# Signalsmith-Audio/signalsmith-stretch

Hardware: AMD Instinct MI355X
Metric: Msamples/sec (in+out) at 48kHz stereo presetDefault (higher is better)
Workload: dtype f32

## Files before the change

### signalsmith-stretch_amd/csrc/smst_fft.hip

```cpp
#include "smst_kernels_common.h"
#include <type_traits>

namespace smst {

template <int SIGN>
__device__ __forceinline__ float2 twiddle(const float2 *__restrict__ tw, int idx) {
	float2 w = tw[idx];
	if (SIGN > 0) w.y = -w.y;
	return w;
}

template <int SIGN>
__device__ __forceinline__ void dft4(float2 &a, float2 &b, float2 &c, float2 &d) {
	float2 apc = cadd(a, c), amc = csub(a, c), bpd = cadd(b, d), bmd = csub(b, d);
	float2 jb = (SIGN < 0) ? mulNegI(bmd) : mulI(bmd);
	a = cadd(apc, bpd);
	b = cadd(amc, jb);
	c = csub(apc, bpd);
	d = csub(amc, jb);
}
template <int SIGN>
__device__ __forceinline__ void dft3(float2 &a, float2 &b, float2 &c) {
	const float s3 = 0.86602540378443864676f;
	float2 bpc = cadd(b, c), bmc = csub(b, c);
	float2 t = make_float2(a.x - 0.5f*bpc.x, a.y - 0.5f*bpc.y);
	float2 u = cscale((SIGN < 0) ? mulNegI(bmc) : mulI(bmc), s3);
	a = cadd(a, bpc);
	b = cadd(t, u);
	c = csub(t, u);
}
template <int SIGN>
__device__ __forceinline__ void dft5(float2 &a, float2 &b, float2 &c, float2 &d, float2 &e) {
	const float c1 = 0.30901699437494742410f, c2 = -0.80901699437494742410f;
	const float s1 = 0.95105651629515357212f, s2 = 0.58778525229247312917f;
	float2 bpe = cadd(b, e), bme = csub(b, e), cpd = cadd(c, d), cmd = csub(c, d);
	float2 t1 = make_float2(a.x + c1*bpe.x + c2*cpd.x, a.y + c1*bpe.y + c2*cpd.y);
	float2 t2 = make_float2(a.x + c2*bpe.x + c1*cpd.x, a.y + c2*bpe.y + c1*cpd.y);
	float2 u1 = make_float2(s1*bme.x + s2*cmd.x, s1*bme.y + s2*cmd.y);
	float2 u2 = make_float2(s2*bme.x - s1*cmd.x, s2*bme.y - s1*cmd.y);
	float2 ju1 = (SIGN < 0) ? mulNegI(u1) : mulI(u1);
	float2 ju2 = (SIGN < 0) ? mulNegI(u2) : mulI(u2);
	a = cadd(a, cadd(bpe, cpd));
	b = cadd(t1, ju1);
	c = cadd(t2, ju2);
	d = csub(t2, ju2);
	e = csub(t1, ju1);
}
template <int SIGN>
__device__ float2 *fftLds(float2 *src, float2 *dst, const FftPlan &plan, const float2 *__restrict__ tw) {
	const int H = plan.H;
	int nCur = H;
	int shift = 0;
	for (int pass = 0; pass < plan.npass; ++pass) {
		const int r = plan.radix[pass];
		const int m = nCur/r;
		const int nb = H/r;
		const int twScale = H/nCur;
		if (r == 4) {
			const int s = 1 << shift;
			for (int t = threadIdx.x; t < nb; t += blockDim.x) {
				const int p = t >> shift, q0 = t & (s - 1);
				const float2 *in = src + q0 + (p << shift);
				const int inStride = m << shift;
				float2 *out = dst + q0 + ((4*p) << shift);
				float2 a = in[0], b = in[inStride], c = in[2*inStride], e = in[3*inStride];
				dft4<SIGN>(a, b, c, e);
				const int ti = p*twScale;
				out[0] = a;
				out[s] = cmulPlain(b, twiddle<SIGN>(tw, ti));
				out[2*s] = cmulPlain(c, twiddle<SIGN>(tw, 2*ti));
				out[3*s] = cmulPlain(e, twiddle<SIGN>(tw, 3*ti));
			}
			shift += 2;
		} else if (r == 2) {
			const int s = 1 << shift;
			for (int t = threadIdx.x; t < nb; t += blockDim.x) {
				const int p = t >> shift, q0 = t & (s - 1);
				const float2 *in = src + q0 + (p << shift);
				const int inStride = m << shift;
				float2 *out = dst + q0 + ((2*p) << shift);
				float2 a = in[0], b = in[inStride];
				out[0] = cadd(a, b);
				out[s] = cmulPlain(csub(a, b), twiddle<SIGN>(tw, p*twScale));
			}
			shift += 1;
		} else if (r == 3) {
			const int s = nb;
			for (int t = threadIdx.x; t < nb; t += blockDim.x) {
				float2 a = src[t], b = src[t + s], c = src[t + 2*s];
				dft3<SIGN>(a, b, c);
				dst[t] = a;
				dst[t + s] = b;
				dst[t + 2*s] = c;
			}
		} else {
			const int s = nb;
			for (int t = threadIdx.x; t < nb; t += blockDim.x) {
				float2 a = src[t], b = src[t + s], c = src[t + 2*s], e = src[t + 3*s], f = src[t + 4*s];
				dft5<SIGN>(a, b, c, e, f);
				dst[t] = a;
				dst[t + s] = b;
				dst[t + 2*s] = c;
				dst[t + 3*s] = e;
				dst[t + 4*s] = f;
			}
		}
		__syncthreads();
		float2 *tmp = src; src = dst; dst = tmp;
		nCur = m;
	}
	return src;
}

template <int SIGN>
__device__ __forceinline__ float2 mulConst(float2 v, float re, float im) {
	const float s = (SIGN < 0) ? -im : im;
	return make_float2(v.x*re - v.y*s, v.x*s + v.y*re);
}
template <int SIGN>
__device__ __forceinline__ void dft16(float2 (&v)[16]) {
#pragma unroll
	for (int i = 0; i < 4; ++i) dft4<SIGN>(v[i], v[i + 4], v[i + 8], v[i + 12]);
	const float c1 = 0.92387953251128675613f, s1 = 0.38268343236508977173f, h = 0.70710678118654752440f;
	v[1 + 4] = mulConst<SIGN>(v[1 + 4], c1, s1);
	v[1 + 8] = mulConst<SIGN>(v[1 + 8], h, h);
	v[1 + 12] = mulConst<SIGN>(v[1 + 12], s1, c1);
	v[2 + 4] = mulConst<SIGN>(v[2 + 4], h, h);
	v[2 + 8] = (SIGN < 0) ? mulNegI(v[2 + 8]) : mulI(v[2 + 8]);
	v[2 + 12] = mulConst<SIGN>(v[2 + 12], -h, h);
	v[3 + 4] = mulConst<SIGN>(v[3 + 4], s1, c1);
	v[3 + 8] = mulConst<SIGN>(v[3 + 8], -h, h);
	v[3 + 12] = mulConst<SIGN>(v[3 + 12], -c1, -s1);
#pragma unroll
	for (int e = 0; e < 4; ++e) dft4<SIGN>(v[4*e], v[4*e + 1], v[4*e + 2], v[4*e + 3]);
}
template <int SIGN, int RA, int N>
__device__ __forceinline__ void dftPow2(float2 (&v)[N], int base, int stride) {
	if constexpr (RA == 2) {
		const float2 a = v[base], b = v[base + stride];
		v[base] = cadd(a, b);
		v[base + stride] = csub(a, b);
	} else if constexpr (RA == 4) {
		dft4<SIGN>(v[base], v[base + stride], v[base + 2*stride], v[base + 3*stride]);
	} else {
		static_assert(RA == 8, "radix 2, 4 or 8");
		float2 e0 = v[base], e1 = v[base + 2*stride], e2 = v[base + 4*stride], e3 = v[base + 6*stride];
		float2 o0 = v[base + stride], o1 = v[base + 3*stride], o2 = v[base + 5*stride], o3 = v[base + 7*stride];
		dft4<SIGN>(e0, e1, e2, e3);
		dft4<SIGN>(o0, o1, o2, o3);
		const float h = 0.70710678118654752440f;
		o1 = mulConst<SIGN>(o1, h, h);
		o2 = (SIGN < 0) ? mulNegI(o2) : mulI(o2);
		o3 = mulConst<SIGN>(o3, -h, h);
		v[base] = cadd(e0, o0); v[base + 4*stride] = csub(e0, o0);
		v[base + stride] = cadd(e1, o1); v[base + 5*stride] = csub(e1, o1);
		v[base + 2*stride] = cadd(e2, o2); v[base + 6*stride] = csub(e2, o2);
		v[base + 3*stride] = cadd(e3, o3); v[base + 7*stride] = csub(e3, o3);
	}
}
template <int R3> struct LastStage {
	static constexpr int G = (R3%3 == 0) ? 3 : 5;
	static constexpr int RA = R3/G;
	static_assert(R3%G == 0 && (RA == 2 || RA == 4 || RA == 8), "last stage: {2,4,8} x {3,5} points");
};
template <int SIGN, int R3>
__device__ __forceinline__ void dftLast(float2 (&v)[R3]) {
	constexpr int G = LastStage<R3>::G, RA = LastStage<R3>::RA;
#pragma unroll
	for (int i = 0; i < G; ++i) dftPow2<SIGN, RA>(v, i, G);
#pragma unroll
	for (int i = 1; i < G; ++i) {
#pragma unroll
		for (int e = 1; e < RA; ++e) {
			const float ang = 6.28318530717958647692f*float(i*e)/float(R3);
			v[i + G*e] = mulConst<SIGN>(v[i + G*e], __builtin_cosf(ang), __builtin_sinf(ang));
		}
	}
#pragma unroll
	for (int e = 0; e < RA; ++e) {
		if constexpr (G == 3) dft3<SIGN>(v[G*e], v[G*e + 1], v[G*e + 2]);
		else dft5<SIGN>(v[G*e], v[G*e + 1], v[G*e + 2], v[G*e + 3 < R3 ? G*e + 3 : 0], v[G*e + 4 < R3 ? G*e + 4 : 0]);
	}
}

struct BlockSync { __device__ __forceinline__ void operator()() const { __syncthreads(); } };
struct NoHook { __device__ __forceinline__ void operator()() const {} };
struct NoArrival { __device__ __forceinline__ float2 operator()(float2 v, int) const { return v; } };
template <int SIGN, int R3, bool LEAN, int ROUNDS = 0, typename Load, typename Prep, typename Store, typename Sync = BlockSync, typename LastRead = NoHook,
          typename Requested = NoHook, typename FirstWritten = NoHook, typename Arrived = NoArrival>
__device__ __forceinline__ void fftFast(float2 *lds, const float4 *__restrict__ twA, const float4 *__restrict__ twB, Load load, Prep prep, Store store,
                                        const int t = threadIdx.x, Sync sync = Sync(), LastRead lastRead = LastRead(), Requested requested = Requested(),
                                        FirstWritten firstWritten = FirstWritten(), Arrived arrived = Arrived()) {
	constexpr int MA = 16*R3;
	float2 v[16];
	if (t < MA) {
#pragma unroll
		for (int k = 0; k < 16; ++k) v[k] = load(t + MA*k, k);
	}
	requested();
	if (t < MA) {
#pragma unroll
		for (int k = 0; k < 16; ++k) v[k] = arrived(v[k], t + MA*k);
		float2 w[16];
		if constexpr (LEAN) {
			const float4 a = twA[t], b = twA[MA + t], c = twA[2*MA + t];
			const float sg = (SIGN > 0) ? -1.0f : 1.0f;
			w[1] = make_float2(a.x, sg*a.y); w[2] = make_float2(a.z, sg*a.w); w[3] = make_float2(b.x, sg*b.y); w[4] = make_float2(b.z, sg*b.w);
			w[8] = make_float2(c.x, sg*c.y); w[12] = make_float2(c.z, sg*c.w);
#pragma unroll
			for (int hi = 4; hi <= 12; hi += 4) {
#pragma unroll
				for (int lo = 1; lo < 4; ++lo) w[hi + lo] = cmulPlain(w[hi], w[lo]);
			}
		} else {
			float4 wA[8];
#pragma unroll
			for (int i = 0; i < 8; ++i) wA[i] = twA[i*MA + t];
#pragma unroll
			for (int n = 1; n < 16; ++n) {
				const float4 pr = wA[(n - 1) >> 1];
				w[n] = ((n - 1) & 1) ? make_float2(pr.z, pr.w) : make_float2(pr.x, pr.y);
				if (SIGN > 0) w[n].y = -w[n].y;
			}
		}
		dft16<SIGN>(v);
#pragma unroll
		for (int pos = 0; pos < 16; ++pos) {
			const int n = (pos >> 2) + 4*(pos & 3);
			float2 val = v[pos];
			if (n > 0) val = cmulPlain(val, w[n]);
			lds[17*t + n] = val;
		}
	}
	firstWritten();
	sync();
	const int p = t >> 4, q0 = t & 15;
	if (t < MA) {
#pragma unroll
		for (int k = 0; k < 16; ++k) v[k] = lds[q0 + 17*(p + R3*k)];
	}
	sync();
	if (t < MA) {
		float4 wB[8];
#pragma unroll
		for (int i = 0; i < 8; ++i) wB[i] = twB[i*R3 + p];
		dft16<SIGN>(v);
#pragma unroll
		for (int pos = 0; pos < 16; ++pos) {
			const int n = (pos >> 2) + 4*(pos & 3);
			float2 val = v[pos];
			if (n > 0) {
				const float4 pr = wB[(n - 1) >> 1];
				float2 w = ((n - 1) & 1) ? make_float2(pr.z, pr.w) : make_float2(pr.x, pr.y);
				if (SIGN > 0) w.y = -w.y;
				val = cmulPlain(val, w);
			}
			lds[q0 + 256*p + 16*n] = val;
		}
	}
	sync();
	if (t < 256) {
		constexpr int G = LastStage<R3>::G, RA = LastStage<R3>::RA;
		float2 u[R3];
#pragma unroll
		for (int k = 0; k < R3; ++k) u[k] = lds[t + 256*k];
		lastRead();
		constexpr int CHUNK = ROUNDS ? R3/ROUNDS : (R3 <= 12 ? R3 : (R3 == 24 ? 6 : 5));
		decltype(prep(0, 0)) ready[CHUNK];
#pragma unroll
		for (int i = 0; i < CHUNK; ++i) {
			const int e = i/G, c = i - G*e;
			ready[i] = prep(t + 256*(e + RA*c), e + RA*c);
		}
		dftLast<SIGN, R3>(u);
#pragma unroll
		for (int p0 = 0; p0 < R3; p0 += CHUNK) {
			if (p0 > 0) {
#pragma unroll
				for (int i = 0; i < CHUNK; ++i) {
					const int pos = p0 + i, e = pos/G, c = pos - G*e;
					if (pos < R3) ready[i] = prep(t + 256*(e + RA*c), e + RA*c);
				}
			}
#pragma unroll
			for (int i = 0; i < CHUNK; ++i) {
				const int pos = p0 + i, e = pos/G, c = pos - G*e;
				if (pos < R3) store(t + 256*(e + RA*c), u[pos], ready[i], e + RA*c);
			}
		}
	}
}

constexpr int fastBlockThreads(int R3) { return 16*R3 > 256 ? 16*R3 : 256; }

__device__ __forceinline__ bool hopWantsAnalysis(const HopDesc &hd, int which) {
	return (hd.flags & HOP_ACTIVE) && (hd.flags & HOP_NEW_SPECTRUM) && !(hd.flags & HOP_PREANALYSED) && (!which || (hd.flags & HOP_REANALYSE_PREV));
}

__device__ __forceinline__ int halfBinIndex(int j, int H, int N) {
	const int kk = 2*j;
	return kk >= H ? N - 1 - kk : kk;
}
__device__ __forceinline__ float2 loadHalfBin(const float2 *X, int j, int H, int N) {
	float2 v = X[halfBinIndex(j, H, N)];
	if (2*j >= H) v.y = -v.y;
	return v;
}
__device__ __forceinline__ void storeHalfBin(float2 *dst, int j, float2 u, int H, int N) {
	const int kk = 2*j;
	if (kk < H) dst[kk] = u;
	else dst[N - 1 - kk] = cconj(u);
}

__device__ __forceinline__ float2 analysisElement(float4 w, const float *x0, const float *x1, int m, int slot) {
	float2 r = make_float2(0.f, 0.f);
	if (slot < 15) { const float xr = x0[m]; r = make_float2(xr*w.x, xr*w.y); }
	if (slot > 0) { const float xi = x1[m]; r = make_float2(fmaf(xi, w.z, r.x), fmaf(xi, w.w, r.y)); }
	return r;
}
__device__ __forceinline__ float2 leanModulation(float2 hb, int k, int per) {
	const float ang = 3.14159265358979323846f*float(k)/float(per);
	return cmulPlain(hb, make_float2(__builtin_cosf(ang), -__builtin_sinf(ang)));
}
__device__ __forceinline__ void storeWindowed(float *dst, int m, float2 u, float2 tw, float wRe, float wIm, int B, int H) {
	const int halfB = B/2;
	const float2 v = cmulcPlain(u, tw);
	if (m < B - halfB) dst[m + halfB] = (2*v.x)*wRe;
	if (m >= H - halfB) dst[m - H + halfB] = (2*v.y)*wIm;
}
__device__ __forceinline__ void storeWindowed(float *dst, int m, float2 u, float4 r, int B, int H) {
	storeWindowed(dst, m, u, make_float2(r.x, r.y), r.z, r.w, B, H);
}

template <int R3, bool LEAN>
__global__ __launch_bounds__(fastBlockThreads(R3)) __attribute__((amdgpu_waves_per_eu(4, 4))) void kAnalyseFast(DevBatch d, IoArgs io, int sBase, int hopBase, int lateOnly) {
	extern __shared__ __attribute__((aligned(16))) unsigned char smemRaw[];
	float2 *lds = reinterpret_cast<float2 *>(smemRaw);
	const BlockCoord bc = xcdAwareBlock();
	const int k = bc.x;
	const int c = bc.y >> 1;
	const int which = bc.y & 1;
	const int s = bc.s;
	const HopDesc hd = d.hops[(size_t)(sBase + s)*d.hopStride + hopBase + k];
	if (!hopWantsAnalysis(hd, which)) return;
	if (lateOnly && analysisWindowInCall(d.B, d.M, d.I, hd.inputOffset, which, io.inSamples[sBase + s])) return;
	const int B = d.B, H = d.M, halfB = B/2, N = d.N;
	const int base = hd.inputOffset - (which ? d.I : 0) - B;
	const float *x = io.in + (size_t)(sBase + s)*io.inStreamStride + (size_t)c*io.inChannelStride;
	const float *hist = d.hist + ((size_t)(sBase + s)*d.C + c)*(size_t)d.histPitch + d.histBase[d.histCur][sBase + s] + d.histLen;
	const float2 *__restrict__ winA = d.winA, *__restrict__ winB = d.winB;
	float2 *dst = (which ? d.Xprev : d.Xcur) + rowOf(d, s, k, c);
	auto prep = [](int, int) { return 0; };
	auto store = [&](int j, float2 u, int, int) { storeHalfBin(dst, j, u, H, N); };
	constexpr int MA = 16*R3;
	const float4 *__restrict__ twA = LEAN ? d.twA6 : d.twA4;
	const float2 *__restrict__ win2 = d.win2;
	const float2 hb = LEAN ? d.halfTw[min((int)threadIdx.x, MA - 1)] : make_float2(0.f, 0.f);
	if (base >= 0 && H - halfB == MA && B - halfB == 15*MA) {
		const float *x0 = x + base + halfB, *x1 = x + base - H + halfB;
		const float4 *__restrict__ win4 = d.win4;
		fftFast<-1, R3, LEAN>(lds, twA, d.twB4,
			[&](int m, int slot) {
				if constexpr (LEAN) {
					const float2 w = win2[m];
					float2 z = make_float2(0.f, 0.f);
					if (slot < 15) z.x = x0[m]*w.x;
					if (slot > 0) z.y = x1[m]*w.y;
					return cmulPlain(z, leanModulation(hb, slot, 32));
				} else {
					return analysisElement(win4[m], x0, x1, m, slot);
				}
			}, prep, store);
		return;
	}
	fftFast<-1, R3, LEAN>(lds, twA, d.twB4,
		[&](int m, int slot) {
			float xr = 0, xi = 0;
			if (m < B - halfB) { int src = base + m + halfB; xr = (src >= 0) ? x[src] : hist[src]; }
			if (m >= H - halfB) { int src = base + m - H + halfB; xi = (src >= 0) ? x[src] : hist[src]; }
			if constexpr (LEAN) {
				const float2 w = win2[m];
				return cmulPlain(make_float2(xr*w.x, xi*w.y), leanModulation(hb, slot, 32));
			} else {
				const float2 a = winA[m], b = winB[m];
				return make_float2(fmaf(xi, b.x, xr*a.x), fmaf(xi, b.y, xr*a.y));
			}
		}, prep, store);
}

struct TeamSync {
	volatile int *word;
	int *generation;
	__device__ __forceinline__ void operator()() const {
		asm volatile("" ::: "memory");
		__builtin_amdgcn_wave_barrier();
		if ((threadIdx.x & 63) == 0) (void)__hip_atomic_fetch_add(const_cast<int *>(word), 1, __ATOMIC_RELAXED, __HIP_MEMORY_SCOPE_WORKGROUP);
		*generation += 4;
		while (__hip_atomic_load(const_cast<int *>(word), __ATOMIC_RELAXED, __HIP_MEMORY_SCOPE_WORKGROUP) < *generation) __builtin_amdgcn_s_sleep(1);
		__builtin_amdgcn_wave_barrier();
		asm volatile("" ::: "memory");
	}
};
template <int R3, int TEAMS>
struct TeamWorkgroup {
	static_assert(16*R3 <= 256, "a team is 256 threads");
	static constexpr int MA = 16*R3, H = 256*R3;
	float4 *table, *twA, *twB;
	float2 *lds;
	int team, t;
	volatile int *word;
	int generation = 0;
	__device__ __forceinline__ TeamWorkgroup(unsigned char *smem, const DevBatch &d, const float4 *__restrict__ source) {
		team = __builtin_amdgcn_readfirstlane(threadIdx.x >> 8);
		t = threadIdx.x & 255;
		table = reinterpret_cast<float4 *>(smem);
		twA = table + H;
		twB = twA + 8*MA;
		lds = reinterpret_cast<float2 *>(twB + 8*R3) + (size_t)team*(H + H/16);
		volatile int *words = reinterpret_cast<volatile int *>(reinterpret_cast<float2 *>(twB + 8*R3) + (size_t)TEAMS*(H + H/16));
		for (int i = threadIdx.x; i < H; i += blockDim.x) table[i] = source[i];
		for (int i = threadIdx.x; i < 8*MA; i += blockDim.x) twA[i] = d.twA4[i];
		for (int i = threadIdx.x; i < 8*R3; i += blockDim.x) twB[i] = d.twB4[i];
		if (threadIdx.x < 16) words[threadIdx.x] = 0;
		__syncthreads();
		word = words + team;
	}
	TeamWorkgroup(const TeamWorkgroup &) = delete;
	__device__ __forceinline__ TeamSync sync() { return TeamSync{word, &generation}; }
};

template <int R3, int TEAMS, bool EXACT>
__global__ __launch_bounds__(256*TEAMS) void kAnalyseTeams(DevBatch d, IoArgs io, const HopDesc *__restrict__ hopTable, int sBase, int hopBase, int tileHops, int nStreams) {
	extern __shared__ __attribute__((aligned(16))) unsigned char smemRaw[];
	constexpr int MA = 16*R3, H = 256*R3, N = 2*H;
	const int B = EXACT ? 480*R3 : d.B, halfB = B/2;
	const int total = tileHops*2*d.C*nStreams;
	TeamWorkgroup<R3, TEAMS> wg(smemRaw, d, d.win4);
	const TeamSync sync = wg.sync();
	const int t = wg.t, tA = t < MA ? t : 0;
	const int stride = gridDim.x*TEAMS;
	for (int lin = blockIdx.x + gridDim.x*wg.team; lin < total; lin += stride) {
		const BlockCoord bc = xcdAwareCoord(lin, tileHops, 2*d.C, nStreams);
		const HopDesc hd = hopTable[(size_t)(sBase + bc.s)*d.hopStride + hopBase + bc.x];
		const int c = bc.y >> 1, which = bc.y & 1;
		if (!hopWantsAnalysis(hd, which) || !analysisWindowInCall(B, H, d.I, hd.inputOffset, which, io.inSamples[sBase + bc.s])) continue;
		const int base = hd.inputOffset - (which ? d.I : 0) - B;
		const float *x = io.in + (size_t)(sBase + bc.s)*io.inStreamStride + (size_t)c*io.inChannelStride;
		const float *x0 = x + base + halfB, *x1 = x + base - H + halfB;
		float2 *dst = (which ? d.Xprev : d.Xcur) + rowOf(d, bc.s, bc.x, c);
		fftFast<-1, R3, false>(wg.lds, wg.twA, wg.twB,
			[&](int m, int slot) { return analysisElement(wg.table[tA + MA*slot], x0, x1, m, slot); },
			[](int, int) { return 0; },
			[&](int j, float2 u, int, int) { storeHalfBin(dst, j, u, H, N); }, t, sync);
		sync();
	}
}

template <int R3, bool LEAN>
__global__ __launch_bounds__(fastBlockThreads(R3)) void kSynthFast(DevBatch d, int sBase, int hopBase) {
	extern __shared__ __attribute__((aligned(16))) unsigned char smemRaw[];
	float2 *lds = reinterpret_cast<float2 *>(smemRaw);
	const int k = blockIdx.x, c = blockIdx.y, s = blockIdx.z;
	const HopDesc hd = d.hops[(size_t)(sBase + s)*d.hopStride + hopBase + k];
	if (!(hd.flags & HOP_ACTIVE)) return;
	const int B = d.B, H = d.M, N = d.N;
	const float2 *X = d.OUT + rowOf(d, s, k, c);
	float *__restrict__ frame = frameOf(d, s, k, c);
	auto loadBin = [&](int j, int) { return loadHalfBin(X, j, H, N); };
	if constexpr (LEAN) {
		const float2 *__restrict__ win2 = d.win2;
		const float2 hb = d.halfTw[min((int)threadIdx.x, 255)];
		fftFast<+1, R3, true>(lds, d.twA6, d.twB4, loadBin,
			[&](int m, int) { return win2[m]; },
			[&](int m, float2 u, float2 w, int j) { storeWindowed(frame, m, u, leanModulation(hb, j, 2*R3), w.x, w.y, B, H); });
	} else {
		const float4 *__restrict__ synTab = d.synTab;
		fftFast<+1, R3, false>(lds, d.twA4, d.twB4, loadBin,
			[&](int m, int) {
				return synTab[m];
			},
			[&](int m, float2 u, float4 r, int) { storeWindowed(frame, m, u, r, B, H); });
	}
}

template <int R3, int TEAMS>
__global__ __launch_bounds__(256*TEAMS) void kSynthTeams(DevBatch d, const HopDesc *__restrict__ hopTable, int sBase, int hopBase, int tileHops, int nStreams) {
	extern __shared__ __attribute__((aligned(16))) unsigned char smemRaw[];
	constexpr int H = 256*R3, N = 2*H;
	const int B = d.B;
	const int total = tileHops*d.C*nStreams;
	TeamWorkgroup<R3, TEAMS> wg(smemRaw, d, d.synTab);
	const TeamSync sync = wg.sync();
	const int stride = gridDim.x*TEAMS;
	for (int lin = blockIdx.x + gridDim.x*wg.team; lin < total; lin += stride) {
		const BlockCoord bc = xcdAwareCoord(lin, tileHops, d.C, nStreams);
		const HopDesc hd = hopTable[(size_t)(sBase + bc.s)*d.hopStride + hopBase + bc.x];
		if (!(hd.flags & HOP_ACTIVE)) continue;
		const float2 *X = d.OUT + rowOf(d, bc.s, bc.x, bc.y);
		float *__restrict__ frame = frameOf(d, bc.s, bc.x, bc.y);
		fftFast<+1, R3, false>(wg.lds, wg.twA, wg.twB,
			[&](int j, int) { return loadHalfBin(X, j, H, N); },
			[&](int m, int) { return wg.table[m]; },
			[&](int m, float2 u, float4 r, int) { storeWindowed(frame, m, u, r, B, H); }, wg.t, sync);
		sync();
	}
}

__device__ __forceinline__ float carriedSumAt(const DevBatch &d, size_t row, int i) { return i < d.carryLen ? loadCarrySum(d, d.carryCur, row + i) : 0.0f; }
__device__ __forceinline__ float carriedProductAt(const DevBatch &d, const float *__restrict__ carryWpOld, int i) { return i < d.carryLen ? carryWpOld[i] : 1e-30f; }
struct FrameRange { int lo, hi; };
__device__ __forceinline__ FrameRange coveringFrames(int relFirst, int relLast, int B, int I, int hopCount) {
	FrameRange r;
	r.hi = (relLast >= 0) ? relLast/I : -1;
	r.lo = (relFirst - B + 1 > 0) ? (relFirst - B + 1 + I - 1)/I : 0;
	if (r.hi > hopCount - 1) r.hi = hopCount - 1;
	return r;
}
__device__ __forceinline__ float windowProductAt(const DevBatch &d, const EmitDesc &ed, const float *__restrict__ carryWpOld, int i) {
	float wp = carriedProductAt(d, carryWpOld, i);
	if (ed.hopCount > 0) {
		const int rel = ed.nLo + i - ed.firstHopPos - d.delta;
		const FrameRange q = coveringFrames(rel, rel, d.B, d.I, ed.hopCount);
		for (int k = q.lo; k <= q.hi; ++k) wp += d.wprod[rel - k*d.I];
	}
	return wp;
}
__global__ __launch_bounds__(256) void kEmitProducts(DevBatch d, int sBase, int tileIndex) {
	const int sg = sBase + blockIdx.y;
	const EmitDesc ed = d.emit[(size_t)sg*d.emitStride + tileIndex];
	const int span = ed.nHi - ed.nLo, CL = d.carryLen;
	const float *carryWpOld = d.carryWp[d.carryCur] + carryWpRow(d, sg) + d.carryBase[d.carryCur][sg];
	const int i = blockIdx.x*blockDim.x + threadIdx.x;
	if (i == 0) d.carryBase[d.carryCur ^ 1][sg] = 0;
	if (i < d.wpHeadLen) d.wpHead[(size_t)sg*d.wpHeadLen + i] = windowProductAt(d, ed, carryWpOld, i);
	else if (i - d.wpHeadLen < CL) d.carryWp[d.carryCur ^ 1][carryWpRow(d, sg) + (i - d.wpHeadLen)] = windowProductAt(d, ed, carryWpOld, span + (i - d.wpHeadLen));
}

template <int R3, int QN, int SLOTS, bool SPLIT>
__global__ __launch_bounds__(512) void kSynthEmitTeams(DevBatch d, IoArgs io, int sBase, int tileIndex, int nStreams) {
	constexpr int TEAMS = 2, MA = 16*R3, H = 256*R3, N = 2*H, NI = QN + 1, DQ = SPLIT ? 1 : 0;
	extern __shared__ __attribute__((aligned(16))) unsigned char smemRaw[];
	const int B = d.B, I = d.I, CL = d.carryLen;
	TeamWorkgroup<R3, TEAMS> wg(smemRaw, d, d.synTab);
	const TeamSync sync = wg.sync();
	const int team = wg.team, t = wg.t;
	float2 *lds = wg.lds;
	float *ex = reinterpret_cast<float *>(lds);
	float steady[SLOTS];
#pragma unroll
	for (int slot = 0; slot < SLOTS; ++slot) {
		const int r = 256*slot + t;
		steady[slot] = 1e-30f;
#pragma unroll
		for (int a = QN - 1; a >= 0; --a) {
			if (r < I && a*I + r < B) steady[slot] += d.wprod[a*I + r];
		}
		keepUnconditional(steady[slot]);
	}
	const int items = nStreams*d.C;
	for (int item = blockIdx.x*TEAMS + team; item < items; item += gridDim.x*TEAMS) {
		const int s = item/d.C, c = item - s*d.C, sg = sBase + s;
		const EmitDesc ed = d.emit[(size_t)sg*d.emitStride + tileIndex];
		const int cnt = ed.hopCount, span = ed.nHi - ed.nLo;
		const int carryFrom = d.carryBase[d.carryCur][sg];
		const size_t carryRow = carrySumRow(d, sg, c), carried = carryRow + carryFrom;
		const float *wpOld = d.carryWp[d.carryCur] + carryWpRow(d, sg) + carryFrom;
		const float *wpHead = d.wpHead + (size_t)sg*d.wpHeadLen;
		float *out = io.out + (size_t)sg*io.outStreamStride + (size_t)c*io.outChannelStride;
		auto place = [&](int n, float sum, float wp) {
			if (n < ed.nHi) out[n] = sum/wp;
			else if (n - ed.nHi < CL) storeCarrySum(d, d.carryCur ^ 1, carryRow + (n - ed.nHi), sum);
		};
		if (cnt == 0) {
			for (int i = t; i < span + CL; i += 256) place(ed.nLo + i, carriedSumAt(d, carried, i), carriedProductAt(d, wpOld, i));
			continue;
		}
		const int off = ed.firstHopPos - ed.nLo;
		for (int i = t; i < off; i += 256) place(ed.nLo + i, carriedSumAt(d, carried, i), carriedProductAt(d, wpOld, i));
		float acc[NI][SLOTS];
#pragma unroll
		for (int u = 0; u < NI; ++u) {
#pragma unroll
			for (int slot = 0; slot < SLOTS; ++slot) {
				const int r = 256*slot + t, i = off + u*I + r;
				acc[u][slot] = r < I ? carriedSumAt(d, carried, i) : 0.0f;
			}
		}
#pragma unroll
		for (int u = 0; u < NI; ++u) {
#pragma unroll
			for (int slot = 0; slot < SLOTS; ++slot) keepUnconditional(acc[u][slot]);
		}
		auto overlapAdd = [&]() {
			float e[QN][SLOTS];
			int tt = t;
			keepUnconditional(tt);
#pragma unroll
			for (int a = 0; a < QN; ++a) {
#pragma unroll
				for (int slot = 0; slot < SLOTS; ++slot) {
					const int r = 256*slot + tt, i = a*I + r;
					e[a][slot] = ex[r < I && i < B ? i : 0];
				}
			}
#pragma unroll
			for (int a = 0; a < QN; ++a) {
#pragma unroll
				for (int slot = 0; slot < SLOTS; ++slot) {
					const int r = 256*slot + t, i = a*I + r;
					keepUnconditional(e[a][slot]);
					acc[a + DQ][slot] = (r < I && i < B) ? acc[a + DQ][slot] + e[a][slot] : acc[a + DQ][slot];
				}
			}
		};
		auto emitInterval = [&](int q) {
			const int n0 = ed.firstHopPos + q*I;
			float wp[SLOTS];
#pragma unroll
			for (int slot = 0; slot < SLOTS; ++slot) wp[slot] = steady[slot];
			if (q < NI) {
				Async4 head[SLOTS];
#pragma unroll
				for (int slot = 0; slot < SLOTS; ++slot) {
					const int r = 256*slot + t;
					asyncLoad4(head[slot], wpHead + (r < I ? off + q*I + r : 0));
				}
				asyncWait<0>();
#pragma unroll
				for (int slot = 0; slot < SLOTS; ++slot) {
					asyncArrived(head[slot]);
					if (256*slot + t < I) wp[slot] = asyncValue(head[slot]);
				}
			}
			if (n0 + I <= ed.nHi) {
#pragma unroll
				for (int slot = 0; slot < SLOTS; ++slot) {
					const int r = 256*slot + t;
					if (r < I) out[n0 + r] = acc[0][slot]/wp[slot];
				}
			} else {
#pragma unroll
				for (int slot = 0; slot < SLOTS; ++slot) {
					const int r = 256*slot + t;
					if (r < I) place(n0 + r, acc[0][slot], wp[slot]);
				}
			}
#pragma unroll
			for (int u = 0; u + 1 < NI; ++u) {
#pragma unroll
				for (int slot = 0; slot < SLOTS; ++slot) acc[u][slot] = acc[u + 1][slot];
			}
#pragma unroll
			for (int slot = 0; slot < SLOTS; ++slot) acc[NI - 1][slot] = 0.0f;
		};
		Async8 next[16];
#pragma unroll
		for (int k = 0; k < 16; ++k) asyncClear(next[k]);
		auto request = [&](int q) {
			const float2 *X = d.OUT + rowOf(d, s, q, c);
			if (t < MA) {
#pragma unroll
				for (int k = 0; k < 16; ++k) asyncLoad8(next[k], X + halfBinIndex(t + MA*k, H, N));
			}
		};
		auto landed = [&]() {
			asyncWait<0>();
#pragma unroll
			for (int k = 0; k < 16; ++k) asyncArrived(next[k]);
		};
		request(0);
		landed();
		for (int q = 0; q < cnt; ++q) {
			fftFast<+1, R3, false, 2>(lds, wg.twA, wg.twB,
				[&](int, int k) { return asyncValue(next[k]); },
				[&](int m, int) { return wg.table[m]; },
				[&](int m, float2 u, float4 r, int) { storeWindowed(ex, m, u, r, B, H); }, t, sync, sync,
				[&]() {
					if (q > 0) overlapAdd();
					sync();
				},
				[&]() {
					if (q > 0) emitInterval(q - 1);
					request(q + 1 < cnt ? q + 1 : q);
				},
				[&](float2 v, int j) { if (2*j >= H) v.y = -v.y; return v; });
			sync();
			landed();
		}
		overlapAdd();
		sync();
		emitInterval(cnt - 1);
		const bool trailing = SPLIT && ed.firstHopPos + cnt*I < ed.nHi;
		if (trailing) emitInterval(cnt);
		const int n0 = ed.firstHopPos + (cnt + (trailing ? 1 : 0))*I;
#pragma unroll
		for (int u = 0; u < NI; ++u) {
#pragma unroll
			for (int slot = 0; slot < SLOTS; ++slot) {
				const int r = 256*slot + t;
				if (r < I) place(n0 + u*I + r, acc[u][slot], 1.0f);
			}
		}
	}
}

__global__ __launch_bounds__(256) void kEnergy(DevBatch d, IoArgs io, int sBase, float *__restrict__ energyOut) {
	const int s = blockIdx.x, part = blockIdx.y, parts = gridDim.y;
	if (part == 0 && (int)threadIdx.x >= parts && (int)threadIdx.x < kEnergyParts) energyOut[(size_t)(sBase + s)*kEnergyParts + threadIdx.x] = 0.0f;
	const int n = io.inSamples[sBase + s];
	const int lo = (int)((long long)n*part/parts), hi = (int)((long long)n*(part + 1)/parts);
	float acc = 0;
	for (int c = 0; c < d.C; ++c) {
		const float *x = io.in + (size_t)(sBase + s)*io.inStreamStride + (size_t)c*io.inChannelStride;
		for (int i = lo + threadIdx.x; i < hi; i += blockDim.x) {
			float v = x[i];
			acc += v*v;
		}
	}
	extern __shared__ __attribute__((aligned(16))) unsigned char smemRaw[];
	float *red = reinterpret_cast<float *>(smemRaw);
	red[threadIdx.x] = acc;
	__syncthreads();
	for (int w = 128; w > 0; w >>= 1) {
		if ((int)threadIdx.x < w) red[threadIdx.x] += red[threadIdx.x + w];
		__syncthreads();
	}
	if (threadIdx.x == 0) energyOut[(size_t)(sBase + s)*kEnergyParts + part] = red[0];
}

template <bool BIG>
__global__ __launch_bounds__(256) void kAnalyse(DevBatch d, IoArgs io, int sBase, int hopBase) {
	extern __shared__ __attribute__((aligned(16))) unsigned char smemRaw[];
	float2 *bufA = reinterpret_cast<float2 *>(smemRaw);
	float2 *bufB = bufA + d.M;

	const BlockCoord bc = xcdAwareBlock();
	const int k = bc.x;
	const int c = bc.y >> 1;
	const int which = bc.y & 1;
	const int s = bc.s;
	const HopDesc hd = d.hops[(size_t)(sBase + s)*d.hopStride + hopBase + k];
	if (!hopWantsAnalysis(hd, which)) return;

	const int B = d.B, H = d.M, halfB = B/2;
	const int base = hd.inputOffset - (which ? d.I : 0) - B;
	const float *x = io.in + (size_t)(sBase + s)*io.inStreamStride + (size_t)c*io.inChannelStride;
	const float *hist = d.hist + ((size_t)(sBase + s)*d.C + c)*(size_t)d.histPitch + d.histBase[d.histCur][sBase + s];
	const float *__restrict__ win = d.window;
	float2 *dst = (which ? d.Xprev : d.Xcur) + rowOf(d, s, k, c);
	if (BIG) bufB = dst;

	for (int m = threadIdx.x; m < H; m += blockDim.x) {
		float re = 0, im = 0;
		if (m < B - halfB) {
			int i = m + halfB;
			int src = base + i;
			float v = (src >= 0) ? x[src] : hist[d.histLen + src];
			re = v*win[i];
		}
		if (m >= H - halfB) {
			int i = m - H + halfB;
			int src = base + i;
			float v = (src >= 0) ? x[src] : hist[d.histLen + src];
			im = v*win[i];
		}
		bufA[m] = cmulPlain(make_float2(re, im), d.halfTw[m]);
	}
	__syncthreads();
	float2 *res = fftLds<-1>(bufA, bufB, d.plan, d.twH);
	if (BIG && res == dst) {
		for (int j = threadIdx.x; j < H; j += blockDim.x) bufA[j] = dst[j];
		__syncthreads();
		res = bufA;
	}
	const int N = d.N;
	for (int j = threadIdx.x; j < H; j += blockDim.x) storeHalfBin(dst, j, res[j], H, N);
}

template <bool BIG>
__global__ __launch_bounds__(256) void kSynth(DevBatch d, int sBase, int hopBase) {
	extern __shared__ __attribute__((aligned(16))) unsigned char smemRaw[];
	float2 *bufA = reinterpret_cast<float2 *>(smemRaw);
	float2 *bufB = bufA + d.M;
	const int k = blockIdx.x, c = blockIdx.y, s = blockIdx.z;
	if (BIG) bufB = d.fftScratch + rowOf(d, s, k, c);
	const HopDesc hd = d.hops[(size_t)(sBase + s)*d.hopStride + hopBase + k];
	if (!(hd.flags & HOP_ACTIVE)) return;
	const int B = d.B, H = d.M, N = d.N, halfB = B/2;
	const float2 *X = d.OUT + rowOf(d, s, k, c);
	for (int j = threadIdx.x; j < H; j += blockDim.x) bufA[j] = loadHalfBin(X, j, H, N);
	__syncthreads();
	float2 *res = fftLds<+1>(bufA, bufB, d.plan, d.twH);
	float *frame = frameOf(d, s, k, c);
	const float *__restrict__ win = d.window;
	for (int m = threadIdx.x; m < H; m += blockDim.x) {
		const float wRe = (m < B - halfB) ? win[m + halfB] : 0.0f, wIm = (m >= H - halfB) ? win[m - H + halfB] : 0.0f;
		storeWindowed(frame, m, res[m], d.halfTw[m], wRe, wIm, B, H);
	}
}

template <int KMAX>
__global__ __launch_bounds__(256) void kEmit(DevBatch d, IoArgs io, int sBase, int tileIndex) {
	const int s = blockIdx.z, sg = sBase + s, c = blockIdx.y;
	const EmitDesc ed = d.emit[(size_t)sg*d.emitStride + tileIndex];
	const int span = ed.nHi - ed.nLo;
	const int i0 = 4*(blockIdx.x*blockDim.x + threadIdx.x);
	const int CL = d.carryLen;
	const int total = span + CL;
	if (i0 >= total) return;
	const int B = d.B, I = d.I;
	const int carryFrom = d.carryBase[d.carryCur][sg];
	const size_t carryRow = carrySumRow(d, sg, c);
	const float *carryWpOld = d.carryWp[d.carryCur] + carryWpRow(d, sg) + carryFrom;
	if (i0 == 0 && c == 0) d.carryBase[d.carryCur ^ 1][sg] = 0;
	float sum[4], wp[4];
	if (i0 + 3 < CL && !d.halfState) {
		const float4 a = *reinterpret_cast<const float4 *>(d.carrySum[d.carryCur] + carryRow + carryFrom + i0), b = *reinterpret_cast<const float4 *>(carryWpOld + i0);
		sum[0] = a.x; sum[1] = a.y; sum[2] = a.z; sum[3] = a.w;
		wp[0] = b.x; wp[1] = b.y; wp[2] = b.z; wp[3] = b.w;
	} else {
#pragma unroll
		for (int j = 0; j < 4; ++j) {
			const int i = i0 + j;
			sum[j] = carriedSumAt(d, carryRow + carryFrom, i);
			wp[j] = carriedProductAt(d, carryWpOld, i);
		}
	}
	if (ed.hopCount > 0) {
		const int rel0 = ed.nLo + i0 - ed.firstHopPos - d.delta;
		const FrameRange cover = coveringFrames(rel0, rel0 + 3, B, I, ed.hopCount);
		const int qLo = cover.lo, qHi = cover.hi;
		float4 f[KMAX], w[KMAX];
		bool fast[KMAX];
#pragma unroll
		for (int k = 0; k < KMAX; ++k) {
			const int q = qLo + k, idx0 = rel0 - q*I;
			fast[k] = q <= qHi && idx0 >= 0 && idx0 + 3 < B;
			const float *frame = frameOf(d, s, fast[k] ? q : 0, c);
			f[k] = *reinterpret_cast<const float4 *>(frame + (fast[k] ? idx0 : 0));
			w[k] = *reinterpret_cast<const float4 *>(d.wprod + (fast[k] ? idx0 : 0));
		}
#pragma unroll
		for (int k = 0; k < KMAX; ++k) {
			const int q = qLo + k, idx0 = rel0 - q*I;
			if (fast[k]) {
				sum[0] += f[k].x; sum[1] += f[k].y; sum[2] += f[k].z; sum[3] += f[k].w;
				wp[0] += w[k].x; wp[1] += w[k].y; wp[2] += w[k].z; wp[3] += w[k].w;
			} else if (q <= qHi) {
				const float *frame = frameOf(d, s, q, c);
#pragma unroll
				for (int j = 0; j < 4; ++j) {
					const int idx = idx0 + j;
					if (idx >= 0 && idx < B) { sum[j] += frame[idx]; wp[j] += d.wprod[idx]; }
				}
			}
		}
		for (int q = qLo + KMAX; q <= qHi; ++q) {
			const int idx0 = rel0 - q*I;
			const float *frame = frameOf(d, s, q, c);
#pragma unroll
			for (int j = 0; j < 4; ++j) {
				const int idx = idx0 + j;
				if (idx >= 0 && idx < B) { sum[j] += frame[idx]; wp[j] += d.wprod[idx]; }
			}
		}
	}
	float *out = io.out + (size_t)sg*io.outStreamStride + (size_t)c*io.outChannelStride + ed.nLo;
	if (i0 + 3 < span) {
		*reinterpret_cast<float4 *>(out + i0) = make_float4(sum[0]/wp[0], sum[1]/wp[1], sum[2]/wp[2], sum[3]/wp[3]);
	} else {
#pragma unroll
		for (int j = 0; j < 4; ++j) {
			const int i = i0 + j;
			if (i < span) {
				out[i] = sum[j]/wp[j];
			} else if (i < total) {
				storeCarrySum(d, d.carryCur ^ 1, carryRow + (i - span), sum[j]);
				if (c == 0) d.carryWp[d.carryCur ^ 1][carryWpRow(d, sg) + (i - span)] = wp[j];
			}
		}
	}
}

__global__ __launch_bounds__(256) void kEmitCarried(DevBatch d, IoArgs io) {
	const int sg = blockIdx.x;
	const EmitDesc ed = d.emit[(size_t)sg*d.emitStride];
	const int span = ed.nHi - ed.nLo, from = d.carryBase[d.carryCur][sg];
	const float *wpRow = d.carryWp[d.carryCur] + carryWpRow(d, sg) + from;
	for (int c = 0; c < d.C; ++c) {
		const size_t row = carrySumRow(d, sg, c) + from;
		float *out = io.out + (size_t)sg*io.outStreamStride + (size_t)c*io.outChannelStride + ed.nLo;
		for (int i = threadIdx.x; i < span; i += blockDim.x) {
			out[i] = carriedSumAt(d, row, i)/carriedProductAt(d, wpRow, i);
		}
	}
	__syncthreads();
	if (threadIdx.x == 0) d.carryBase[d.carryCur][sg] = from + span;
}

void launchEnergy(const DevBatch &d, const IoArgs &io, int sBase, int nStreams, int maxSamples, float *energyOut, hipStream_t st) {
	const int parts = std::max(1, std::min(kEnergyParts, maxSamples/1024));
	hipLaunchKernelGGL(kEnergy, dim3(nStreams, parts), dim3(256), 256*sizeof(float), st, d, io, sBase, energyOut);
}
template <int... R3S, typename F>
static bool withR3(int M, F f) { return ((M == 256*R3S && (f(std::integral_constant<int, R3S>()), true)) || ...); }
template <typename F> static bool withFastR3(int M, F f) { return withR3<10, 12, 20, 24>(M, f); }
template <typename F> static bool withTeamR3(int M, F f) { return withR3<10, 12>(M, f); }
template <typename F>
static void withFlag(bool flag, F f) {
	if (flag) f(std::true_type()); else f(std::false_type());
}
static size_t fastLdsBytes(int M) { return ((size_t)M + M/16)*sizeof(float2); }
static size_t teamLdsBytes(int M, int teams) {
	return ((size_t)M + M/2 + M/32)*sizeof(float4) + teams*fastLdsBytes(M) + 64;
}
static bool fastApplies(const DevBatch &d) { return !d.noFastFft && isFastSize(d.M); }
static bool teamsAvailable(const DevBatch &d) { return fastApplies(d) && withTeamR3(d.M, [](auto) {}) && d.fftTeams && !d.fftLean; }
static bool teamsApply(const DevBatch &d, int jobs) { return teamsAvailable(d) && (d.fftTeams == 2 || jobs >= 6*d.teamsGrid); }
static int teamsWorkgroups(const DevBatch &d, int jobs) {
	return std::max(8, std::min((jobs + 2)/3/8*8, d.teamsGrid));
}
constexpr int synthEmitQN(int R3) { return R3 == 10 ? 3 : 4; }
constexpr int synthEmitSlots(int R3) { return R3 == 10 ? 8 : 6; }

void launchAnalyse(const DevBatch &d, const IoArgs &io, int sBase, int nStreams, int hopBase, int tileHops, bool anyInCall, bool anyLate, hipStream_t st) {
	const dim3 grid(tileHops, d.C*2, nStreams);
	const int jobs = tileHops*d.C*2*nStreams;
	const bool teams = anyInCall && teamsApply(d, jobs);
	if (teams) {
		const WindowPad pad = windowPad(d.B, d.M);
		withTeamR3(d.M, [&](auto r3) { withFlag(pad.lo == 0 && pad.hi == 0, [&](auto exact) {
			hipLaunchKernelGGL((kAnalyseTeams<r3.value, 3, exact.value>), dim3(teamsWorkgroups(d, jobs)), dim3(768), teamLdsBytes(d.M, 3), st, d, io, d.hops, sBase, hopBase, tileHops, nStreams);
		}); });
		countLaunch(LK_ANALYSE_TEAMS);
		if (!anyLate) return;
	}
	const int lateOnly = teams ? 1 : 0;
	countLaunch(fastApplies(d) ? LK_ANALYSE_FAST : LK_ANALYSE_GENERIC);
	if (!d.noFastFft && withFastR3(d.M, [&](auto r3) { withFlag(d.fftLean != 0, [&](auto lean) {
			hipLaunchKernelGGL((kAnalyseFast<r3.value, lean.value>), grid, dim3(fastBlockThreads(r3.value)), fastLdsBytes(d.M), st, d, io, sBase, hopBase, lateOnly);
		}); })) return;
	size_t lds = 2*(size_t)d.M*sizeof(float2);
	if (fftNeedsScratch(d.M)) hipLaunchKernelGGL(kAnalyse<true>, grid, dim3(256), lds/2, st, d, io, sBase, hopBase);
	else hipLaunchKernelGGL(kAnalyse<false>, grid, dim3(256), lds, st, d, io, sBase, hopBase);
}
void launchSynth(const DevBatch &d, int sBase, int nStreams, int hopBase, int tileHops, hipStream_t st) {
	const dim3 grid(tileHops, d.C, nStreams);
	const int jobs = tileHops*d.C*nStreams;
	if (teamsApply(d, jobs)) {
		withTeamR3(d.M, [&](auto r3) {
			hipLaunchKernelGGL((kSynthTeams<r3.value, 3>), dim3(teamsWorkgroups(d, jobs)), dim3(768), teamLdsBytes(d.M, 3), st, d, d.hops, sBase, hopBase, tileHops, nStreams);
		});
		countLaunch(LK_SYNTH_TEAMS);
		return;
	}
	countLaunch(fastApplies(d) ? LK_SYNTH_FAST : LK_SYNTH_GENERIC);
	if (!d.noFastFft && withFastR3(d.M, [&](auto r3) { withFlag(d.fftLean != 0, [&](auto lean) {
			hipLaunchKernelGGL((kSynthFast<r3.value, lean.value>), grid, dim3(fastBlockThreads(r3.value)), fastLdsBytes(d.M), st, d, sBase, hopBase);
		}); })) return;
	size_t lds = 2*(size_t)d.M*sizeof(float2);
	if (fftNeedsScratch(d.M)) hipLaunchKernelGGL(kSynth<true>, grid, dim3(256), lds/2, st, d, sBase, hopBase);
	else hipLaunchKernelGGL(kSynth<false>, grid, dim3(256), lds, st, d, sBase, hopBase);
}
bool synthEmitApplies(const DevBatch &d, int nStreams, int tileHops) {
	if (!teamsAvailable(d) || !d.synthEmit) return false;
	if (!(d.delta == 0 || d.delta == d.I)) return false;
	const int QN = synthEmitQN(d.M/256), SLOTS = synthEmitSlots(d.M/256);
	if (QN*d.I < d.B || d.I > 256*SLOTS || d.B > d.N) return false;
	if ((QN + 2)*d.I > d.wpHeadLen) return false;
	return d.synthEmit == 2 || (tileHops >= 8 && nStreams*d.C >= 64);
}
void launchEmitProducts(const DevBatch &d, int sBase, int nStreams, int tileIndex, hipStream_t st) {
	hipLaunchKernelGGL(kEmitProducts, dim3(divUp(d.wpHeadLen + d.carryLen, 256), nStreams), dim3(256), 0, st, d, sBase, tileIndex);
}
void launchSynthEmit(const DevBatch &d, const IoArgs &io, int sBase, int nStreams, int tileIndex, hipStream_t st) {
	const int items = nStreams*d.C;
	const int wgs = std::min(divUp(items, 2), d.teamsGrid);
	withTeamR3(d.M, [&](auto r3) { withFlag(d.delta != 0, [&](auto split) {
		hipLaunchKernelGGL((kSynthEmitTeams<r3.value, synthEmitQN(r3.value), synthEmitSlots(r3.value), split.value>), dim3(wgs), dim3(512), teamLdsBytes(d.M, 2), st, d, io, sBase, tileIndex, nStreams);
	}); });
	countLaunch(LK_SYNTH_EMIT);
}
void launchEmit(const DevBatch &d, const IoArgs &io, int sBase, int nStreams, int tileIndex, int maxSpan, hipStream_t st) {
	const dim3 grid(divUp(divUp(maxSpan + d.carryLen, 4), 256), d.C, nStreams);
	const int covering = divUp(d.B + 3, d.I);
	if (covering <= 3) hipLaunchKernelGGL(kEmit<3>, grid, dim3(256), 0, st, d, io, sBase, tileIndex);
	else if (covering <= 4) hipLaunchKernelGGL(kEmit<4>, grid, dim3(256), 0, st, d, io, sBase, tileIndex);
	else if (covering <= 5) hipLaunchKernelGGL(kEmit<5>, grid, dim3(256), 0, st, d, io, sBase, tileIndex);
	else hipLaunchKernelGGL(kEmit<6>, grid, dim3(256), 0, st, d, io, sBase, tileIndex);
}
void launchEmitCarried(const DevBatch &d, const IoArgs &io, hipStream_t st) {
	hipLaunchKernelGGL(kEmitCarried, dim3(d.S), dim3(256), 0, st, d, io);
	countLaunch(LK_EMIT_CARRIED);
}

}
```

Baseline: 45760.

## Specialize synth-emit kernel on compile-time hop geometry and trim live registers

```diff
diff --git a/signalsmith-stretch_amd/csrc/smst_fft.hip b/signalsmith-stretch_amd/csrc/smst_fft.hip
--- a/signalsmith-stretch_amd/csrc/smst_fft.hip
+++ b/signalsmith-stretch_amd/csrc/smst_fft.hip
@@ -536,61 +536,85 @@
 	else if (i - d.wpHeadLen < CL) d.carryWp[d.carryCur ^ 1][carryWpRow(d, sg) + (i - d.wpHeadLen)] = windowProductAt(d, ed, carryWpOld, span + (i - d.wpHeadLen));
 }
 
-template <int R3, int QN, int SLOTS, bool SPLIT>
+struct SynthEmitEdge {
+	EmitDesc ed;
+	float *out;
+	size_t carryRow;
+	size_t carried;
+	const float *wpOld;
+};
+__device__ __forceinline__ SynthEmitEdge synthEmitEdge(const DevBatch &d, const IoArgs &io, int sg, int c, int tileIndex) {
+	SynthEmitEdge e;
+	e.ed = d.emit[(size_t)sg*d.emitStride + tileIndex];
+	const int carryFrom = d.carryBase[d.carryCur][sg];
+	e.carryRow = carrySumRow(d, sg, c);
+	e.carried = e.carryRow + carryFrom;
+	e.wpOld = d.carryWp[d.carryCur] + carryWpRow(d, sg) + carryFrom;
+	e.out = io.out + (size_t)sg*io.outStreamStride + (size_t)c*io.outChannelStride;
+	return e;
+}
+__device__ __forceinline__ void synthEmitPlace(const DevBatch &d, const SynthEmitEdge &e, int n, float sum, float wp) {
+	if (n < e.ed.nHi) e.out[n] = sum/wp;
+	else if (n - e.ed.nHi < d.carryLen) storeCarrySum(d, d.carryCur ^ 1, e.carryRow + (n - e.ed.nHi), sum);
+}
+template <int R3, int QN, int SLOTS, bool SPLIT, int GI, int GB>
 __global__ __launch_bounds__(512) void kSynthEmitTeams(DevBatch d, IoArgs io, int sBase, int tileIndex, int nStreams) {
 	constexpr int TEAMS = 2, MA = 16*R3, H = 256*R3, N = 2*H, NI = QN + 1, DQ = SPLIT ? 1 : 0;
+	static_assert(GI == 0 || (GI <= 256*SLOTS && GI > 256*(SLOTS - 1) && QN*GI >= GB && GB <= N), "the geometry this instantiation is for");
 	extern __shared__ __attribute__((aligned(16))) unsigned char smemRaw[];
-	const int B = d.B, I = d.I, CL = d.carryLen;
+	const int B = GI ? GB : d.B, I = GI ? GI : d.I;
 	TeamWorkgroup<R3, TEAMS> wg(smemRaw, d, d.synTab);
 	const TeamSync sync = wg.sync();
 	const int team = wg.team, t = wg.t;
 	float2 *lds = wg.lds;
 	float *ex = reinterpret_cast<float *>(lds);
+	auto inInterval = [&](int slot) { return 256*slot + t < I; };
+	auto inFrame = [&](int a, int slot) { return 256*slot + t < I && a*I + 256*slot + t < B; };
 	float steady[SLOTS];
 #pragma unroll
 	for (int slot = 0; slot < SLOTS; ++slot) {
-		const int r = 256*slot + t;
 		steady[slot] = 1e-30f;
 #pragma unroll
 		for (int a = QN - 1; a >= 0; --a) {
-			if (r < I && a*I + r < B) steady[slot] += d.wprod[a*I + r];
+			if (inFrame(a, slot)) steady[slot] += d.wprod[a*I + 256*slot + t];
 		}
 		keepUnconditional(steady[slot]);
 	}
-	const int items = nStreams*d.C;
+	const int C = d.C, items = nStreams*C;
+	const unsigned hopPitch = (unsigned)C*(unsigned)d.Mp;
 	for (int item = blockIdx.x*TEAMS + team; item < items; item += gridDim.x*TEAMS) {
-		const int s = item/d.C, c = item - s*d.C, sg = sBase + s;
-		const EmitDesc ed = d.emit[(size_t)sg*d.emitStride + tileIndex];
-		const int cnt = ed.hopCount, span = ed.nHi - ed.nLo;
-		const int carryFrom = d.carryBase[d.carryCur][sg];
-		const size_t carryRow = carrySumRow(d, sg, c), carried = carryRow + carryFrom;
-		const float *wpOld = d.carryWp[d.carryCur] + carryWpRow(d, sg) + carryFrom;
-		const float *wpHead = d.wpHead + (size_t)sg*d.wpHeadLen;
-		float *out = io.out + (size_t)sg*io.outStreamStride + (size_t)c*io.outChannelStride;
-		auto place = [&](int n, float sum, float wp) {
-			if (n < ed.nHi) out[n] = sum/wp;
-			else if (n - ed.nHi < CL) storeCarrySum(d, d.carryCur ^ 1, carryRow + (n - ed.nHi), sum);
-		};
-		if (cnt == 0) {
-			for (int i = t; i < span + CL; i += 256) place(ed.nLo + i, carriedSumAt(d, carried, i), carriedProductAt(d, wpOld, i));
-			continue;
-		}
-		const int off = ed.firstHopPos - ed.nLo;
-		for (int i = t; i < off; i += 256) place(ed.nLo + i, carriedSumAt(d, carried, i), carriedProductAt(d, wpOld, i));
+		const int s = item/C, c = item - s*C, sg = sBase + s;
+		int cnt, off, firstHopPos;
 		float acc[NI][SLOTS];
+		{
+			const SynthEmitEdge e = synthEmitEdge(d, io, sg, c, tileIndex);
+			const int CL = d.carryLen;
+			cnt = e.ed.hopCount;
+			if (cnt == 0) {
+				const int span = e.ed.nHi - e.ed.nLo;
+				for (int i = t; i < span + CL; i += 256) synthEmitPlace(d, e, e.ed.nLo + i, carriedSumAt(d, e.carried, i), carriedProductAt(d, e.wpOld, i));
+				continue;
+			}
+			firstHopPos = e.ed.firstHopPos;
+			off = firstHopPos - e.ed.nLo;
+			for (int i = t; i < off; i += 256) synthEmitPlace(d, e, e.ed.nLo + i, carriedSumAt(d, e.carried, i), carriedProductAt(d, e.wpOld, i));
+#pragma unroll
+			for (int u = 0; u < NI; ++u) {
+#pragma unroll
+				for (int slot = 0; slot < SLOTS; ++slot) {
+					const int i = off + u*I + 256*slot + t;
+					acc[u][slot] = inInterval(slot) ? carriedSumAt(d, e.carried, i) : 0.0f;
+				}
+			}
+		}
 #pragma unroll
 		for (int u = 0; u < NI; ++u) {
 #pragma unroll
-			for (int slot = 0; slot < SLOTS; ++slot) {
-				const int r = 256*slot + t, i = off + u*I + r;
-				acc[u][slot] = r < I ? carriedSumAt(d, carried, i) : 0.0f;
-			}
-		}
-#pragma unroll
-		for (int u = 0; u < NI; ++u) {
-#pragma unroll
 			for (int slot = 0; slot < SLOTS; ++slot) keepUnconditional(acc[u][slot]);
 		}
+		const float2 *spectra = d.OUT + rowOf(d, s, 0, c);
+		float *outHops = io.out + (size_t)sg*io.outStreamStride + (size_t)c*io.outChannelStride + firstHopPos;
+		const float *wpHead = d.wpHead + (size_t)sg*d.wpHeadLen + off;
 		auto overlapAdd = [&]() {
 			float e[QN][SLOTS];
 			int tt = t;
@@ -599,65 +623,60 @@
 			for (int a = 0; a < QN; ++a) {
 #pragma unroll
 				for (int slot = 0; slot < SLOTS; ++slot) {
-					const int r = 256*slot + tt, i = a*I + r;
-					e[a][slot] = ex[r < I && i < B ? i : 0];
+					if (GI && (256*slot >= GI || a*GI + 256*slot >= GB)) continue;
+					e[a][slot] = ex[inFrame(a, slot) ? a*I + 256*slot + tt : 0];
 				}
 			}
 #pragma unroll
 			for (int a = 0; a < QN; ++a) {
 #pragma unroll
 				for (int slot = 0; slot < SLOTS; ++slot) {
-					const int r = 256*slot + t, i = a*I + r;
+					if (GI && (256*slot >= GI || a*GI + 256*slot >= GB)) continue;
 					keepUnconditional(e[a][slot]);
-					acc[a + DQ][slot] = (r < I && i < B) ? acc[a + DQ][slot] + e[a][slot] : acc[a + DQ][slot];
+					acc[a + DQ][slot] = inFrame(a, slot) ? acc[a + DQ][slot] + e[a][slot] : acc[a + DQ][slot];
 				}
 			}
 		};
-		auto emitInterval = [&](int q) {
-			const int n0 = ed.firstHopPos + q*I;
-			float wp[SLOTS];
+		auto moveRing = [&]() {
+#pragma unroll
+			for (int u = 0; u + 1 < NI; ++u) {
+#pragma unroll
+				for (int slot = 0; slot < SLOTS; ++slot) acc[u][slot] = acc[u + 1][slot];
+			}
+#pragma unroll
+			for (int slot = 0; slot < SLOTS; ++slot) acc[NI - 1][slot] = 0.0f;
+		};
+		auto productsOf = [&](int q, float (&wp)[SLOTS]) {
 #pragma unroll
 			for (int slot = 0; slot < SLOTS; ++slot) wp[slot] = steady[slot];
 			if (q < NI) {
 				Async4 head[SLOTS];
-#pragma unroll
-				for (int slot = 0; slot < SLOTS; ++slot) {
-					const int r = 256*slot + t;
-					asyncLoad4(head[slot], wpHead + (r < I ? off + q*I + r : 0));
-				}
+				const float *from = wpHead + q*I;
+#pragma unroll
+				for (int slot = 0; slot < SLOTS; ++slot) asyncLoad4(head[slot], from + (inInterval(slot) ? 256*slot + t : 0));
 				asyncWait<0>();
 #pragma unroll
 				for (int slot = 0; slot < SLOTS; ++slot) {
 					asyncArrived(head[slot]);
-					if (256*slot + t < I) wp[slot] = asyncValue(head[slot]);
+					if (inInterval(slot)) wp[slot] = asyncValue(head[slot]);
 				}
 			}
-			if (n0 + I <= ed.nHi) {
-#pragma unroll
-				for (int slot = 0; slot < SLOTS; ++slot) {
-					const int r = 256*slot + t;
-					if (r < I) out[n0 + r] = acc[0][slot]/wp[slot];
-				}
-			} else {
-#pragma unroll
-				for (int slot = 0; slot < SLOTS; ++slot) {
-					const int r = 256*slot + t;
-					if (r < I) place(n0 + r, acc[0][slot], wp[slot]);
-				}
-			}
-#pragma unroll
-			for (int u = 0; u + 1 < NI; ++u) {
-#pragma unroll
-				for (int slot = 0; slot < SLOTS; ++slot) acc[u][slot] = acc[u + 1][slot];
-			}
-#pragma unroll
-			for (int slot = 0; slot < SLOTS; ++slot) acc[NI - 1][slot] = 0.0f;
+		};
+		auto emitFinal = [&](int q) {
+			float wp[SLOTS];
+			productsOf(q, wp);
+			float *to = outHops + q*I;
+#pragma unroll
+			for (int slot = 0; slot < SLOTS; ++slot) {
+				if (inInterval(slot)) to[256*slot + t] = acc[0][slot]/wp[slot];
+			}
+			moveRing();
 		};
 		Async8 next[16];
 #pragma unroll
 		for (int k = 0; k < 16; ++k) asyncClear(next[k]);
 		auto request = [&](int q) {
-			const float2 *X = d.OUT + rowOf(d, s, q, c);
+			const float2 *X = spectra + (unsigned)q*hopPitch;
 			if (t < MA) {
 #pragma unroll
 				for (int k = 0; k < 16; ++k) asyncLoad8(next[k], X + halfBinIndex(t + MA*k, H, N));
@@ -680,7 +699,7 @@
 					sync();
 				},
 				[&]() {
-					if (q > 0) emitInterval(q - 1);
+					if (q > 0) emitFinal(q - 1);
 					request(q + 1 < cnt ? q + 1 : q);
 				},
 				[&](float2 v, int j) { if (2*j >= H) v.y = -v.y; return v; });
@@ -689,16 +708,29 @@
 		}
 		overlapAdd();
 		sync();
-		emitInterval(cnt - 1);
-		const bool trailing = SPLIT && ed.firstHopPos + cnt*I < ed.nHi;
-		if (trailing) emitInterval(cnt);
-		const int n0 = ed.firstHopPos + (cnt + (trailing ? 1 : 0))*I;
+		int sgE = sg, cE = c;
+		keepUnconditional(sgE);
+		keepUnconditional(cE);
+		const SynthEmitEdge e = synthEmitEdge(d, io, __builtin_amdgcn_readfirstlane(sgE), __builtin_amdgcn_readfirstlane(cE), tileIndex);
+		auto emitEdge = [&](int q) {
+			float wp[SLOTS];
+			productsOf(q, wp);
+			const int n0 = firstHopPos + q*I;
+#pragma unroll
+			for (int slot = 0; slot < SLOTS; ++slot) {
+				if (inInterval(slot)) synthEmitPlace(d, e, n0 + 256*slot + t, acc[0][slot], wp[slot]);
+			}
+			moveRing();
+		};
+		emitEdge(cnt - 1);
+		const bool trailing = SPLIT && firstHopPos + cnt*I < e.ed.nHi;
+		if (trailing) emitEdge(cnt);
+		const int n0 = firstHopPos + (cnt + (trailing ? 1 : 0))*I;
 #pragma unroll
 		for (int u = 0; u < NI; ++u) {
 #pragma unroll
 			for (int slot = 0; slot < SLOTS; ++slot) {
-				const int r = 256*slot + t;
-				if (r < I) place(n0 + u*I + r, acc[u][slot], 1.0f);
+				if (inInterval(slot)) synthEmitPlace(d, e, n0 + u*I + 256*slot + t, acc[u][slot], 1.0f);
 			}
 		}
 	}
@@ -973,12 +1005,21 @@
 void launchEmitProducts(const DevBatch &d, int sBase, int nStreams, int tileIndex, hipStream_t st) {
 	hipLaunchKernelGGL(kEmitProducts, dim3(divUp(d.wpHeadLen + d.carryLen, 256), nStreams), dim3(256), 0, st, d, sBase, tileIndex);
 }
+template <int GI, int GB> struct SynthEmitGeometry { static constexpr int interval = GI, block = GB, slots = (GI + 255)/256; };
+template <int R3, typename F>
+static void withSynthEmitGeometry(const DevBatch &d, F f) {
+	using Slots = std::integral_constant<int, synthEmitSlots(R3)>;
+	auto is = [&](auto g) { return d.I == g.interval && d.B == g.block && (f(g, std::integral_constant<int, g.slots>()), true); };
+	if constexpr (R3 == 12) { if (is(SynthEmitGeometry<1440, 5760>()) || is(SynthEmitGeometry<1323, 5292>())) return; }
+	if constexpr (R3 == 10) { if (is(SynthEmitGeometry<1920, 4800>()) || is(SynthEmitGeometry<1764, 4410>())) return; }
+	f(SynthEmitGeometry<0, 0>(), Slots());
+}
 void launchSynthEmit(const DevBatch &d, const IoArgs &io, int sBase, int nStreams, int tileIndex, hipStream_t st) {
 	const int items = nStreams*d.C;
 	const int wgs = std::min(divUp(items, 2), d.teamsGrid);
-	withTeamR3(d.M, [&](auto r3) { withFlag(d.delta != 0, [&](auto split) {
-		hipLaunchKernelGGL((kSynthEmitTeams<r3.value, synthEmitQN(r3.value), synthEmitSlots(r3.value), split.value>), dim3(wgs), dim3(512), teamLdsBytes(d.M, 2), st, d, io, sBase, tileIndex, nStreams);
-	}); });
+	withTeamR3(d.M, [&](auto r3) { withFlag(d.delta != 0, [&](auto split) { withSynthEmitGeometry<r3.value>(d, [&](auto g, auto slots) {
+		hipLaunchKernelGGL((kSynthEmitTeams<r3.value, synthEmitQN(r3.value), slots.value, split.value, g.interval, g.block>), dim3(wgs), dim3(512), teamLdsBytes(d.M, 2), st, d, io, sBase, tileIndex, nStreams);
+	}); }); });
 	countLaunch(LK_SYNTH_EMIT);
 }
 void launchEmit(const DevBatch &d, const IoArgs &io, int sBase, int nStreams, int tileIndex, int maxSpan, hipStream_t st) {
```

New measurement: 47410 (median of 6 runs). 1.04x the previous value.
